# gau-nernst/vision-toolbox

Measured on AMD Instinct MI355X. Metric: images/sec (node) CSPDarknet-53 bf16 train step @224px, higher is better.
Workload: dtype bf16; 1 GPU; cspdarknet53 train step (fwd+CE+bwd+allreduce+SGD), batch 256/GPU, 3x224x224, 1000 classes, BASELINE configs[1]; global_batch=256, per_gpu_batch=256, parallelism=dp1, rccl_ranks=1, local_device=cuda:0, hip_graphs=False, main_stream_priority=-1, sync_bn=False, deterministic=False

## Files before the change

### vision-toolbox_amd/csrc/vt_pointwise.hip

```cpp
#include <stdlib.h>
#include <string.h>

#include <hip/hip_ext.h>

#include "vt_common.h"
#include "vt_bn_fin.h"

namespace {

typedef __attribute__((address_space(3))) s16x4 lds_s16x4;
typedef __attribute__((ext_vector_type(8))) short s16x8;

enum { PW_STATS = 0, PW_APPLY = 1, PW_REDUCE = 2, PW_BWD = 3 };

constexpr int pw_depth(int N, int K, int mode) {
#ifdef VT_PW_DEPTH
    return VT_PW_DEPTH;
#else
    return 1;
#endif
}

struct PwArgs {
    const bf16_t* x;
    int ldx;
    long M;
    int N0;
    const bf16_t* w[2];
    int ldw[2];
    bf16_t* y[2];
    const bf16_t* dy[2];
    int ldy[2];
    const bf16_t* res[2];
    int ldr[2];
    float* stats[2];
    const float* coef;
    const float* bcoef[2];
    bf16_t* dx;
    int lddx;
    const bf16_t* add;
    int ldadd;
    float* dw[2];
    int lddw[2];
    bf16_t* dz[2];
    int lddz[2];
    int relu;
    int nunits;
    int Nr, Kr;
    int fin;
    VtFinFwd ffin[2];
    VtFinBwd bfin[2];
    const float* pcoef;
    int pact;
    int pfin_on;
    VtFinFwd pfin;
    float* psums;
};

__device__ __forceinline__ uint4 ldg16(const bf16_t* p) { return *(const uint4*)p; }
__device__ __forceinline__ bf16x8 as_frag(const uint4& v) { return __builtin_bit_cast(bf16x8, v); }
__device__ __forceinline__ f32x4 mma(const bf16x8& a, const bf16x8& b, const f32x4& c) {
    return __builtin_amdgcn_mfma_f32_16x16x32_bf16(a, b, c, 0, 0, 0);
}
__device__ __forceinline__ float bfround(float v) { return (float)(bf16_t)v; }

template <int N, int K>
struct PwGeom {
    static constexpr int NT = N / 16, NU = N / 32, KS = K / 32, CT = K / 16, KV = K / 32;
    static constexpr int PITCH = 2 * K + 16;
    static constexpr int W_BYTES = N * PITCH;
    static constexpr int COEF_OFF = W_BYTES;
    static constexpr int RED_OFF = COEF_OFF + 5 * N * 4;
    static constexpr bool kFull = N * K <= 4096;
#ifndef VT_PW_REGW
#define VT_PW_REGW 2048
#endif
    static constexpr bool kRegW = N * K <= VT_PW_REGW;
    static constexpr int RED_BYTES = (kFull ? N * K * 4 : 0) > 4 * 2 * N * 4 ? N * K * 4 : 4 * 2 * N * 4;
    static constexpr int SMEM = RED_OFF + RED_BYTES;
};

template <int N, int K, int MODE, bool EX, int PROD = 0>
__global__ void __launch_bounds__(256) pw_kernel(const PwArgs a) {
    using G = PwGeom<N, K>;
    constexpr int NT = G::NT, NU = G::NU, KS = G::KS, CT = G::CT, KV = G::KV, PITCH = G::PITCH;
    constexpr bool kDW = (MODE == PW_BWD) && G::kFull;
    constexpr int kDepth = pw_depth(N, K, MODE);
    extern __shared__ __attribute__((aligned(16))) char smem[];
    char* sW = smem;
    float* sCoef = (float*)(smem + G::COEF_OFF);
    float* sRed = (float*)(smem + G::RED_OFF);

    const int tid = threadIdx.x, lane = tid & 63;
    const int wave = __builtin_amdgcn_readfirstlane(tid >> 6);
    const int pl = lane & 15, q = lane >> 4;
    const int N0 = a.N0;

    for (int idx = tid; idx < N * (K / 8); idx += 256) {
        const int n = idx / (K / 8), ch = idx - n * (K / 8);
        const int g = n >= N0;
        const bf16_t* src = a.w[g] + (long)(n - (g ? N0 : 0)) * a.ldw[g] + ch * 8;
        const bool real = n < a.Nr && ch * 8 < a.Kr;
        *(uint4*)(sW + n * PITCH + ch * 16) = real ? ldg16(src) : make_uint4(0, 0, 0, 0);
    }
    bool fin_done = false;
    if constexpr ((MODE == PW_APPLY || MODE == PW_BWD) && N <= 128) {
        if (a.fin) {
            fin_done = true;
            const int w = tid & 1, n = tid >> 1;
            const bool on = n < a.Nr;
            const int g = (on && n >= N0) ? 1 : 0, lc = on ? n - (g ? N0 : 0) : 0;
            if constexpr (MODE == PW_APPLY) {
                const VtFinFwd& f = a.ffin[g];
                const VtFinFwdPre pre = vt_fin_fwd_pre(f, lc);
                const double v = vt_replica_sum<false>(f.stats, (long)w * f.C + lc, 2L * f.C);
                const double o = __shfl_xor(v, 1, 64);
                if (on && w == 0) {
                    float sc, sf;
                    vt_fin_fwd_channel(f, lc, v, o, pre.g, pre.b, pre.rm, pre.rv, sc, sf, blockIdx.x == 0);
                    sCoef[n] = sc, sCoef[N + n] = sf;
                }
            } else {
                const VtFinBwd& f = a.bfin[g];
                const VtFinBwdPre pre = vt_fin_bwd_pre(f, lc);
                const float sh = on ? a.coef[N + n] : 0.f;
                const double v = vt_replica_sum<false>(f.sums, (long)w * f.C + lc, 2L * f.C);
                const double o = __shfl_xor(v, 1, 64);
                if (on && w == 0) {
                    float b, d;
                    vt_fin_bwd_channel(f, lc, v, o, pre.a, pre.mu, pre.istd, pre.dg, pre.db, b, d, blockIdx.x == 0);
                    sCoef[n] = pre.a, sCoef[N + n] = sh, sCoef[2 * N + n] = pre.a, sCoef[3 * N + n] = b, sCoef[4 * N + n] = d;
                }
            }
            for (int i = tid; i < 5 * N; i += 256) {
                const int which = i / N, n2 = i - which * N;
                if (n2 >= a.Nr || which >= (MODE == PW_APPLY ? 2 : 5)) sCoef[i] = 0.f;
// ... 50 lines not shown

    const unsigned za_base = (unsigned)((8 * (pl >> 2) + (pl & 3)) * PITCH + 16 * q);
    const unsigned ta_base = (unsigned)((8 * q + (pl >> 2)) * PITCH + 16 * (pl & 3));
    auto wz_frag = [&](int nt, int s) -> bf16x8 {
        const uint4 v = *(const uint4*)(sW + za_base + (nt >> 1) * 32 * PITCH + (nt & 1) * 4 * PITCH + s * 64);
        return as_frag(v);
    };
    auto wt_frag = [&](int ct, int u) -> bf16x8 {
        const char* p = sW + ta_base + u * 32 * PITCH + (ct >> 1) * 64 + (ct & 1) * 8;
        const s16x4 lo = __builtin_amdgcn_ds_read_tr16_b64_v4i16((lds_s16x4*)p);
        const s16x4 hi = __builtin_amdgcn_ds_read_tr16_b64_v4i16((lds_s16x4*)(p + 4 * PITCH));
        const s16x8 v = {lo[0], lo[1], lo[2], lo[3], hi[0], hi[1], hi[2], hi[3]};
        return __builtin_bit_cast(bf16x8, v);
    };
    bf16x8 wz[G::kRegW ? NT : 1][G::kRegW ? KS : 1];
    bf16x8 wt[(G::kRegW && MODE == PW_BWD) ? CT : 1][(G::kRegW && MODE == PW_BWD) ? NU : 1];
    if constexpr (G::kRegW) {
#pragma unroll
        for (int nt = 0; nt < NT; ++nt)
#pragma unroll
            for (int s = 0; s < KS; ++s) wz[nt][s] = wz_frag(nt, s);
        if constexpr (MODE == PW_BWD) {
#pragma unroll
            for (int ct = 0; ct < CT; ++ct)
#pragma unroll
                for (int u = 0; u < NU; ++u) wt[ct][u] = wt_frag(ct, u);
        }
    }
    bf16x8 sel[2];
    if constexpr (kDW) {
#pragma unroll
        for (int tt = 0; tt < 2; ++tt) {
            s16x8 v;
#pragma unroll
            for (int j = 0; j < 8; ++j) v[j] = (8 * q + j == 16 * tt + pl) ? (short)0x3F80 : (short)0;
            sel[tt] = __builtin_bit_cast(bf16x8, v);
        }
    }

    float s1[NU][8], s2[NU][8];
    if constexpr (MODE == PW_STATS || MODE == PW_REDUCE) {
#pragma unroll
        for (int u = 0; u < NU; ++u)
#pragma unroll
            for (int e = 0; e < 8; ++e) s1[u][e] = s2[u][e] = 0.f;
    }
    f32x4 dwacc[kDW ? NT : 1][kDW ? CT : 1];
    if constexpr (kDW) {
#pragma unroll
        for (int nt = 0; nt < NT; ++nt)
#pragma unroll
            for (int ct = 0; ct < CT; ++ct) dwacc[nt][ct] = f32x4{0.f, 0.f, 0.f, 0.f};
    }
    float p1[kPRed ? KV : 1][8], p2[kPRed ? KV : 1][8];
    if constexpr (kPRed) {
#pragma unroll
        for (int v = 0; v < KV; ++v)
#pragma unroll
            for (int e = 0; e < 8; ++e) p1[v][e] = p2[v][e] = 0.f;
    }

    struct Regs {
        uint4 x[KS];
        uint4 dy[(MODE >= PW_REDUCE) ? NU : 1];
        uint4 ex[(MODE == PW_APPLY) ? NU : (MODE == PW_BWD ? KV : 1)];
    };
    auto group_of = [&](int u) -> int { return 32 * u >= N0; };

    auto load_unit = [&](Regs& r, int unit) {
        const long p = (long)unit * 16 + pl;
        const long pc = p < a.M ? p : a.M - 1;
#pragma unroll
        for (int s = 0; s < KS; ++s) r.x[s] = ldg16(a.x + pc * a.ldx + (32 * s + 8 * q < a.Kr ? 32 * s + 8 * q : 0));
        if constexpr (MODE >= PW_REDUCE) {
#pragma unroll
            for (int u = 0; u < NU; ++u) {
                const int g = group_of(u);
                r.dy[u] = ldg16(a.dy[g] + pc * a.ldy[g] + (32 * u - (g ? N0 : 0)) + 8 * q);
            }
        }
        if constexpr (MODE == PW_APPLY) {
#pragma unroll
            for (int u = 0; u < NU; ++u) {
                const int g = group_of(u);
                if constexpr (EX)
                    r.ex[u] = ldg16(a.res[g] + pc * a.ldr[g] + (32 * u + 8 * q < a.Nr ? (32 * u - (g ? N0 : 0)) + 8 * q : 0));
            }
        }
        if constexpr (MODE == PW_BWD) {
            if constexpr (EX) {
#pragma unroll
                for (int v = 0; v < KV; ++v) r.ex[v] = ldg16(a.add + pc * a.ldadd + 32 * v + 8 * q);
            }
        }
    };

    auto compute_unit = [&](const Regs& r, int unit) {
        asm volatile("" ::: "memory");
        const long p = (long)unit * 16 + pl;
        const bool ok = p < a.M;
        uint4 xn[PROD ? KS : 1];
        if constexpr (PROD) {
#pragma unroll
            for (int s = 0; s < KS; ++s) {
                float v[8], psc[8], psf[8];
                const int ck = 32 * s + 8 * q;
                *(f32x4*)&psc[0] = *(const f32x4*)(sProd + ck);
                *(f32x4*)&psc[4] = *(const f32x4*)(sProd + ck + 4);
                *(f32x4*)&psf[0] = *(const f32x4*)(sProd + K + ck);
                *(f32x4*)&psf[4] = *(const f32x4*)(sProd + K + ck + 4);
                VecIO<bf16_t>::unpack(r.x[s], v);
#pragma unroll
                for (int e = 0; e < 8; ++e) {
                    v[e] = fmaf(v[e], psc[e], psf[e]);
                    v[e] = a.pact ? fmaxf(v[e], 0.f) : v[e];
                }
                xn[s] = VecIO<bf16_t>::pack(v);
            }
        }
        const uint4* xop = PROD ? xn : r.x;
        f32x4 zacc[NT];
#pragma unroll
        for (int nt = 0; nt < NT; ++nt) {
            zacc[nt] = f32x4{0.f, 0.f, 0.f, 0.f};
#pragma unroll
            for (int s = 0; s < KS; ++s) {
                const bf16x8 A = G::kRegW ? wz[G::kRegW ? nt : 0][G::kRegW ? s : 0] : wz_frag(nt, s);
                zacc[nt] = mma(A, as_frag(xop[s]), zacc[nt]);
            }
        }
        bf16x8 dzt[(MODE == PW_BWD) ? NU : 1];
#pragma unroll
        for (int u = 0; u < NU; ++u) {
            float z[8];
#pragma unroll
            for (int e = 0; e < 8; ++e) z[e] = bfround(zacc[2 * u + (e >> 2)][e & 3]);
            const int cb = 32 * u + 8 * q;
            if constexpr (MODE == PW_STATS) {
#pragma unroll
                for (int e = 0; e < 8; ++e) {
                    const float zz = ok ? z[e] : 0.f;
                    s1[u][e] += zz;
                    s2[u][e] = fmaf(zz, zz, s2[u][e]);
                }
            } else {
                float sc[8], sf[8];
                *(f32x4*)&sc[0] = *(const f32x4*)(sCoef + cb);
                *(f32x4*)&sc[4] = *(const f32x4*)(sCoef + cb + 4);
                *(f32x4*)&sf[0] = *(const f32x4*)(sCoef + N + cb);
                *(f32x4*)&sf[4] = *(const f32x4*)(sCoef + N + cb + 4);
                if constexpr (MODE == PW_APPLY) {
                    const int g = group_of(u);
                    float v[8], rr[8];
#pragma unroll
                    for (int e = 0; e < 8; ++e) rr[e] = 0.f;
                    if constexpr (EX) VecIO<bf16_t>::unpack(r.ex[u], rr);
#pragma unroll
                    for (int e = 0; e < 8; ++e) {
                        v[e] = fmaf(z[e], sc[e], sf[e]);
                        v[e] = a.relu ? fmaxf(v[e], 0.f) : v[e];
                        v[e] += rr[e];
                    }
                    if (ok && 32 * u + 8 * q < a.Nr)
                        *(uint4*)(a.y[g] + p * a.ldy[g] + (32 * u - (g ? N0 : 0)) + 8 * q) = VecIO<bf16_t>::pack(v);
                } else {
                    float gy[8];
                    VecIO<bf16_t>::unpack(r.dy[u], gy);
// ... 3 lines not shown
                        float mu[8];
                        *(f32x4*)&mu[0] = *(const f32x4*)(sCoef + 2 * N + cb);
                        *(f32x4*)&mu[4] = *(const f32x4*)(sCoef + 2 * N + cb + 4);
#pragma unroll
                        for (int e = 0; e < 8; ++e) {
                            s1[u][e] += gy[e];
                            s2[u][e] = fmaf(gy[e], z[e] - mu[e], s2[u][e]);
                        }
                    } else {
                        float ca[8], cbb[8], cd[8], dz[8];
                        *(f32x4*)&ca[0] = *(const f32x4*)(sCoef + 2 * N + cb);
                        *(f32x4*)&ca[4] = *(const f32x4*)(sCoef + 2 * N + cb + 4);
                        *(f32x4*)&cbb[0] = *(const f32x4*)(sCoef + 3 * N + cb);
                        *(f32x4*)&cbb[4] = *(const f32x4*)(sCoef + 3 * N + cb + 4);
                        *(f32x4*)&cd[0] = *(const f32x4*)(sCoef + 4 * N + cb);
                        *(f32x4*)&cd[4] = *(const f32x4*)(sCoef + 4 * N + cb + 4);
#pragma unroll
                        for (int e = 0; e < 8; ++e) {
                            dz[e] = fmaf(ca[e], gy[e], fmaf(-cbb[e], z[e], cd[e]));
                            dz[e] = ok ? dz[e] : 0.f;
                        }
                        const uint4 dzp = VecIO<bf16_t>::pack(dz);
                        dzt[u] = as_frag(dzp);
                        if constexpr (!kDW) {
                            const int g = group_of(u);
                            if (a.dz[g] && ok) *(uint4*)(a.dz[g] + p * a.lddz[g] + (32 * u - (g ? N0 : 0)) + 8 * q) = dzp;
                        }
                    }
                }
            }
        }
        if constexpr (MODE == PW_BWD) {
#pragma unroll
            for (int v = 0; v < KV; ++v) {
                f32x4 xa[2];
#pragma unroll
                for (int h = 0; h < 2; ++h) {
                    xa[h] = f32x4{0.f, 0.f, 0.f, 0.f};
#pragma unroll
                    for (int u = 0; u < NU; ++u) {
                        const bf16x8 A = G::kRegW ? wt[G::kRegW ? 2 * v + h : 0][G::kRegW ? u : 0] : wt_frag(2 * v + h, u);
                        xa[h] = mma(A, dzt[u], xa[h]);
                    }
                }
                float o[8], ad[8];
#pragma unroll
                for (int e = 0; e < 8; ++e) ad[e] = 0.f;
                if constexpr (EX) VecIO<bf16_t>::unpack(r.ex[v], ad);
#pragma unroll
                for (int e = 0; e < 8; ++e) o[e] = xa[e >> 2][e & 3] + ad[e];
                const uint4 dxp = VecIO<bf16_t>::pack(o);
                if (ok) *(uint4*)(a.dx + p * a.lddx + 32 * v + 8 * q) = dxp;
                if constexpr (kPRed) {
                    float gq[8], z0[8], psc[8], psf[8], pmu[8];
                    const int ck = 32 * v + 8 * q;
                    *(f32x4*)&psc[0] = *(const f32x4*)(sProd + ck);
                    *(f32x4*)&psc[4] = *(const f32x4*)(sProd + ck + 4);
                    *(f32x4*)&psf[0] = *(const f32x4*)(sProd + K + ck);
                    *(f32x4*)&psf[4] = *(const f32x4*)(sProd + K + ck + 4);
                    *(f32x4*)&pmu[0] = *(const f32x4*)(sProd + 2 * K + ck);
                    *(f32x4*)&pmu[4] = *(const f32x4*)(sProd + 2 * K + ck + 4);
                    VecIO<bf16_t>::unpack(dxp, gq);
                    VecIO<bf16_t>::unpack(r.x[v], z0);
#pragma unroll
                    for (int e = 0; e < 8; ++e) {
                        const float gg = (ok && (!a.pact || fmaf(z0[e], psc[e], psf[e]) > 0.f)) ? gq[e] : 0.f;
                        p1[v][e] += gg;
                        p2[v][e] = fmaf(gg, z0[e] - pmu[e], p2[v][e]);
                    }
                }
            }
        }
        if constexpr (kDW) {
            s16x4 dzT[NT], xT[CT];
            const f32x4 z4 = f32x4{0.f, 0.f, 0.f, 0.f};
#pragma unroll
            for (int nt = 0; nt < NT; ++nt) {
                const f32x4 t0 = mma(dzt[nt >> 1], sel[nt & 1], z4);
                const uint32_t lo = VecIO<bf16_t>::pack2(t0[0], t0[1]), hi = VecIO<bf16_t>::pack2(t0[2], t0[3]);
                dzT[nt] = __builtin_bit_cast(s16x4, make_uint2(lo, hi));
            }
#pragma unroll
            for (int ct = 0; ct < CT; ++ct) {
                const f32x4 t0 = mma(as_frag(xop[ct >> 1]), sel[ct & 1], z4);
                const uint32_t lo = VecIO<bf16_t>::pack2(t0[0], t0[1]), hi = VecIO<bf16_t>::pack2(t0[2], t0[3]);
                xT[ct] = __builtin_bit_cast(s16x4, make_uint2(lo, hi));
            }
#pragma unroll
            for (int nt = 0; nt < NT; ++nt)
#pragma unroll
                for (int ct = 0; ct < CT; ++ct)
                    dwacc[nt][ct] = __builtin_amdgcn_mfma_f32_16x16x16bf16_1k(dzT[nt], xT[ct], dwacc[nt][ct], 0, 0, 0);
        }
    };

    const int stride = (int)gridDim.x * 4;
    const int first = (int)blockIdx.x * 4 + wave;
    const int T = first < a.nunits ? (a.nunits - first + stride - 1) / stride : 0;
    if (T > 0) {
        auto unit_of = [&](int i) { return first + (i < T ? i : T - 1) * stride; };
        Regs ring[kDepth + 1];
#pragma unroll
        for (int j = 0; j < kDepth; ++j) load_unit(ring[j], unit_of(j));
        int i = 0;
        for (; i + kDepth + 1 <= T; i += kDepth + 1) {
#pragma unroll
            for (int j = 0; j <= kDepth; ++j) {
                load_unit(ring[(j + kDepth) % (kDepth + 1)], unit_of(i + j + kDepth));
                compute_unit(ring[j], first + (i + j) * stride);
            }
        }
#pragma unroll
        for (int j = 0; j < kDepth; ++j)
            if (i + j < T) compute_unit(ring[j], first + (i + j) * stride);
    }

    if constexpr (MODE == PW_STATS || MODE == PW_REDUCE) {
#pragma unroll
        for (int u = 0; u < NU; ++u)
#pragma unroll
            for (int e = 0; e < 8; ++e) {
#pragma unroll
                for (int off = 1; off < 16; off <<= 1) {
                    s1[u][e] += __shfl_xor(s1[u][e], off, 64);
                    s2[u][e] += __shfl_xor(s2[u][e], off, 64);
                }
            }
        if (pl == 0) {
#pragma unroll
            for (int u = 0; u < NU; ++u)
#pragma unroll
                for (int e = 0; e < 8; ++e) {
                    sRed[(wave * 2 + 0) * N + 32 * u + 8 * q + e] = s1[u][e];
                    sRed[(wave * 2 + 1) * N + 32 * u + 8 * q + e] = s2[u][e];
                }
        }
        __syncthreads();
        const int rep = (int)(blockIdx.x % kStatReplicas);
        for (int i = tid; i < 2 * N; i += 256) {
            const int which = i / N, n = i - which * N;
            float acc = sRed[(0 * 2 + which) * N + n];
            acc += sRed[(1 * 2 + which) * N + n];
            acc += sRed[(2 * 2 + which) * N + n];
            acc += sRed[(3 * 2 + which) * N + n];
            if (MODE == PW_REDUCE && which) acc *= sCoef[3 * N + n];
            const int g = n >= N0, Cg = g ? N - N0 : N0, c = n - (g ? N0 : 0);
            vt_stat_add(a.stats[g], ((long)rep * 2 + which) * Cg + c, acc);
        }
    }
    if constexpr (kDW) {
#pragma unroll
        for (int nt = 0; nt < NT; ++nt)
#pragma unroll
            for (int ct = 0; ct < CT; ++ct)
#pragma unroll
                for (int r = 0; r < 4; ++r) atomicAdd(&sRed[(16 * nt + 4 * q + r) * K + 16 * ct + pl], dwacc[nt][ct][r]);
        __syncthreads();
        constexpr int NCH = N * K / 256;
        const int rot = (int)((blockIdx.x * 7u) % (unsigned)NCH);
        for (int j = 0; j < NCH; ++j) {
            int ch = j + rot;
            ch -= ch >= NCH ? NCH : 0;
            const int i = ch * 256 + tid;
            const int n = i / K, c = i - n * K;
            const int g = n >= N0;
            float* dst = a.dw[g];
            if (dst) atomicAdd(dst + (long)(n - (g ? N0 : 0)) * a.lddw[g] + c, sRed[i]);
        }
    }
    if constexpr (kPRed) {
#pragma unroll
        for (int v = 0; v < KV; ++v)
#pragma unroll
            for (int e = 0; e < 8; ++e) {
#pragma unroll
                for (int off = 1; off < 16; off <<= 1) {
                    p1[v][e] += __shfl_xor(p1[v][e], off, 64);
                    p2[v][e] += __shfl_xor(p2[v][e], off, 64);
                }
            }
        __syncthreads();
        if (pl == 0) {
#pragma unroll
            for (int v = 0; v < KV; ++v)
#pragma unroll
                for (int e = 0; e < 8; ++e) {
                    sRed[(wave * 2 + 0) * K + 32 * v + 8 * q + e] = p1[v][e];
                    sRed[(wave * 2 + 1) * K + 32 * v + 8 * q + e] = p2[v][e];
                }
        }
        __syncthreads();
        const int rep = (int)(blockIdx.x % kStatReplicas);
        for (int i = tid; i < 2 * K; i += 256) {
            const int which = i / K, c = i - which * K;
            float acc = sRed[(0 * 2 + which) * K + c];
            acc += sRed[(1 * 2 + which) * K + c];
            acc += sRed[(2 * 2 + which) * K + c];
            acc += sRed[(3 * 2 + which) * K + c];
            if (which) acc *= sProd[3 * K + c];
            vt_stat_add(a.psums, ((long)rep * 2 + which) * K + c, acc);
        }
    }
}

template <int N, int K, int MODE, bool EX, int PROD = 0>
int launch_pw(const PwArgs& a, hipStream_t st, const char* who) {
    using G = PwGeom<N, K>;
    auto kern = pw_kernel<N, K, MODE, EX, PROD>;
    constexpr int smem = G::SMEM + (PROD ? 4 * K * 4 : 0);
    static_assert(smem <= 160 * 1024, "weights exceed the LDS of a CU");
    if (smem > 64 * 1024) {
        const int rc = vt_raise_dynamic_lds((const void*)kern, smem, who);
        if (rc != VT_OK) return rc;
    }
    const int knob = (0);
    const int target = knob > 0 ? knob : (a.nunits >= 160000 ? 768 : 512);
    const int per_wave = (8);
    long blocks = ((long)a.nunits + 4 * per_wave - 1) / (4 * per_wave);
    if (blocks > target) blocks = target;
    if (blocks < 1) blocks = 1;
    vt_note_kernel(PROD == 2 ? "pw_kernel<%d,%d,%s,prod+sums>" : PROD ? "pw_kernel<%d,%d,%s,prod>" : "pw_kernel<%d,%d,%s>", N, K, MODE == PW_STATS ? "stats" : MODE == PW_APPLY ? "apply" : MODE == PW_REDUCE ? "reduce" : "bwd");
    VT_LAUNCH_STOP(kern, dim3((unsigned)blocks), dim3(256), smem, st, a);
    VT_CHECK_LAUNCH(who);
    return VT_OK;
}

template <int MODE>
int dispatch_pw(int N, int K, const PwArgs& a, hipStream_t st, const char* who) {
    const bool ex = MODE == PW_APPLY ? a.res[0] != nullptr : (MODE == PW_BWD ? a.add != nullptr : false);
    if (a.pcoef) {
#define VT_PW_PROD_CASE(n, k)                                                      \
    if (N == n && K == k) {                                                        \
        if constexpr (MODE == PW_APPLY || MODE == PW_BWD) {                        \
            if (ex) return launch_pw<n, k, MODE, true, 1>(a, st, who);             \
        }                                                                          \
        if constexpr (MODE == PW_BWD) {                                            \
            if (a.psums) return launch_pw<n, k, MODE, false, 2>(a, st, who);       \
        }                                                                          \
        return launch_pw<n, k, MODE, false, 1>(a, st, who);                        \
    }
        VT_PW_PROD_CASE(32, 32)
        VT_PW_PROD_CASE(64, 64)
        VT_PW_PROD_CASE(32, 64)
#undef VT_PW_PROD_CASE
        vt_set_error("%s: no pointwise kernel with a producer operand for %d -> %d channels", who, K, N);
        return VT_ERR_UNSUPPORTED;
    }
#define VT_PW_CASE(n, k)                                                           \
    if (N == n && K == k) {                                                        \
        if constexpr (MODE == PW_APPLY || MODE == PW_BWD) {                        \
            if (ex) return launch_pw<n, k, MODE, true>(a, st, who);                \
        }                                                                          \
        return launch_pw<n, k, MODE, false>(a, st, who);                           \
    }
    VT_PW_CASE(32, 32)
    VT_PW_CASE(64, 64)
    VT_PW_CASE(32, 64)
    VT_PW_CASE(128, 128)
    VT_PW_CASE(64, 128)
    VT_PW_CASE(160, 160)
    VT_PW_CASE(160, 320)
#undef VT_PW_CASE
// ... 5 lines not shown
    return VT_ERR_UNSUPPORTED;
}

bool shape_ok(int N, int K) {
    return (N == 32 && K == 32) || (N == 64 && K == 64) || (N == 32 && K == 64) || (N == 128 && K == 128) ||
           (N == 64 && K == 128) || (N == 160 && K == 160) || (N == 160 && K == 320);
}

bool ragged_apply_ok(int N, int K, int ngroups) { return ngroups == 1 && N == 80 && (K == 80 || K == 160); }

int fill_common(PwArgs& a, const vt_pw_desc* d, const char* who, bool apply = false) {
    VT_REQUIRE(d, VT_ERR_INVALID, "%s: null descriptor", who);
    VT_REQUIRE(d->dtype == VT_BF16, VT_ERR_UNSUPPORTED, "%s: bf16 only", who);
    VT_REQUIRE(d->M > 0 && d->M < 0x7fffffffL * 16, VT_ERR_INVALID, "%s: bad M", who);
    VT_REQUIRE(d->ngroups == 1 || d->ngroups == 2, VT_ERR_INVALID, "%s: ngroups %d", who, d->ngroups);
    const int N = d->C[0] + (d->ngroups == 2 ? d->C[1] : 0);
    const bool ragged = apply && ragged_apply_ok(N, d->K, d->ngroups);
    VT_REQUIRE(ragged || shape_ok(N, d->K), VT_ERR_UNSUPPORTED, "%s: no pointwise kernel for %d -> %d channels", who, d->K, N);
    VT_REQUIRE(ragged || (d->C[0] > 0 && d->C[0] % 32 == 0 && (d->ngroups == 1 || (d->C[1] > 0 && d->C[1] % 32 == 0))),
               VT_ERR_UNSUPPORTED, "%s: group widths must be multiples of 32", who);
    VT_REQUIRE(d->x && vt_aligned16(d->x) && d->ldx % 8 == 0 && d->ldx >= d->K, VT_ERR_INVALID, "%s: bad x", who);
    VT_REQUIRE(d->M * (int64_t)d->ldx < 0x7fffffff00LL, VT_ERR_UNSUPPORTED, "%s: tensor too large", who);
    memset(&a, 0, sizeof(a));
    a.x = (const bf16_t*)d->x;
    a.ldx = d->ldx;
    a.M = d->M;
    a.N0 = d->C[0];
    a.relu = d->relu;
    a.nunits = (int)((d->M + 15) / 16);
    a.Nr = N, a.Kr = d->K;
    for (int g = 0; g < d->ngroups; ++g) {
        VT_REQUIRE(d->w[g] && vt_aligned16(d->w[g]) && d->ldw[g] % 8 == 0 && d->ldw[g] >= d->K, VT_ERR_INVALID,
                   "%s: bad weights of group %d", who, g);
        a.w[g] = (const bf16_t*)d->w[g];
        a.ldw[g] = d->ldw[g];
    }
    if (d->pcoef) {
        VT_REQUIRE(!ragged && (int64_t)N * d->K <= 4096, VT_ERR_UNSUPPORTED,
                   "%s: a producer operand needs a shape with vt_pw_supported() == 2 (%d -> %d channels)", who, d->K, N);
        VT_REQUIRE(d->pact == 0 || d->pact == 1, VT_ERR_UNSUPPORTED, "%s: producer activation code %d (0 / 1 only)", who, d->pact);
        VT_REQUIRE(vt_aligned16(d->pcoef), VT_ERR_INVALID, "%s: bad producer coefficients", who);
        a.pcoef = d->pcoef;
        a.pact = d->pact;
    }
    return VT_OK;
}

int check_rows(const char* who, const char* what, int g, const void* p, int ld, int C, bool optional) {
    if (!p && optional) return VT_OK;
    VT_REQUIRE(p && vt_aligned16(p) && ld % 8 == 0 && ld >= C, VT_ERR_INVALID, "%s: bad %s of group %d", who, what, g);
    return VT_OK;
}

}

extern "C" {

int vt_pw_supported(int32_t dtype, int32_t K, int32_t C0, int32_t C1) {
    if (dtype != VT_BF16 || C0 <= 0 || C1 < 0 || C0 % 32 != 0 || C1 % 32 != 0) return 0;
    const int N = C0 + C1;
    if (!shape_ok(N, K)) return 0;
    return N * K <= 4096 ? 2 : 1;
}

int vt_pw_apply_supported(int32_t dtype, int32_t K, int32_t C0) {
    return dtype == VT_BF16 && (shape_ok(C0, K) || ragged_apply_ok(C0, K, 1));
}

static int pw_fwd_stats_impl(const vt_pw_desc* d, const vt_bn_fin_fwd* pfin, float* const* stats, void* stream) {
    PwArgs a;
    int rc = fill_common(a, d, "vt_pw_fwd_stats");
    if (rc != VT_OK) return rc;
    for (int g = 0; g < d->ngroups; ++g) {
        VT_REQUIRE(stats && stats[g], VT_ERR_INVALID, "vt_pw_fwd_stats: null statistics buffer");
        a.stats[g] = stats[g];
    }
    if (pfin) {
        float* c = (float*)d->pcoef;
        const int K = d->K;
        a.pfin_on = 1;
        a.pfin = VtFinFwd{pfin->stats, pfin->gamma, pfin->beta, pfin->running_mean, pfin->running_var, pfin->num_batches_tracked,
                          c, c + K, c + 2 * K, c + 3 * K, 1.0 / pfin->count,
                          pfin->count > 1.0 ? pfin->count / (pfin->count - 1.0) : 1.0, pfin->eps, pfin->momentum, K};
    }
    return dispatch_pw<PW_STATS>(a.N0 + (d->ngroups == 2 ? d->C[1] : 0), d->K, a, (hipStream_t)stream, "vt_pw_fwd_stats");
}

int vt_pw_fwd_stats(const vt_pw_desc* d, float* const* stats, void* stream) { return pw_fwd_stats_impl(d, nullptr, stats, stream); }

int vt_pw_fwd_stats_finalize(const vt_pw_desc* d, const vt_bn_fin_fwd* pfin, float* const* stats, void* stream) {
    VT_REQUIRE(d && pfin, VT_ERR_INVALID, "vt_pw_fwd_stats_finalize: null argument");
    VT_REQUIRE(d->pcoef, VT_ERR_INVALID, "vt_pw_fwd_stats_finalize: the descriptor has no producer operand");
    VT_REQUIRE(pfin->stats && pfin->count > 0, VT_ERR_INVALID, "vt_pw_fwd_stats_finalize: bad statistics of the producer");
    VT_REQUIRE((pfin->running_mean == nullptr) == (pfin->running_var == nullptr), VT_ERR_INVALID,
               "vt_pw_fwd_stats_finalize: running_mean/var must both be given or both NULL");
    if (!VT_KNOB("VT_BN_FIN_APPLY", 1)) {
        float* c = (float*)d->pcoef;
        const int K = d->K;
        const int rc = vt_bn_finalize(pfin->stats, K, pfin->count, pfin->gamma, pfin->beta, pfin->eps, pfin->momentum,
                                      pfin->running_mean, pfin->running_var, pfin->num_batches_tracked, c, c + K, c + 2 * K,
                                      c + 3 * K, stream);
        if (rc != VT_OK) return rc;
        return pw_fwd_stats_impl(d, nullptr, stats, stream);
    }
    return pw_fwd_stats_impl(d, pfin, stats, stream);
}
// ... 168 lines not shown
```

### vision-toolbox_amd/csrc/vt_igemm.hip

```cpp
#include <stdlib.h>

#include "vt_common.h"
#include "vt_igemm_args.h"

namespace {

constexpr int kTapBytes = VT_MAX_TAPS * 16;
constexpr int stat_bytes(int WM, int BN) { return WM * 2 * BN * 4 > 2048 ? WM * 2 * BN * 4 : 2048; }

__device__ __attribute__((aligned(16))) unsigned int vt_zero16[4];

__device__ __forceinline__ int swz(int row) { return (0x1320 >> (((row >> 2) & 3) * 4)) & 3; }

__device__ __forceinline__ void glds16(const void* gsrc, unsigned lds_base) {
    unsigned keep;
    asm volatile(
        "s_mov_b32 %0, m0\n\t"
        "s_mov_b32 m0, %2\n\t"
        "s_nop 0\n\t"
        "global_load_lds_dwordx4 %1, off\n\t"
        "s_mov_b32 m0, %0"
        : "=&s"(keep)
        : "v"(gsrc), "s"(lds_base)
        : "memory");
// ... 412 lines not shown
    VT_REQUIRE(d->Cin % epc == 0 && d->Cout % epc == 0 && d->ldx % epc == 0 && d->ldy % epc == 0 &&
                   d->ldw % epc == 0,
               VT_ERR_UNSUPPORTED,
               "vt_conv_igemm: Cin=%d Cout=%d ldx=%d ldy=%d ldw=%d must be multiples of %d", d->Cin,
               d->Cout, d->ldx, d->ldy, d->ldw, epc);
    const bool d2s = (d->flags & VT_CONV_D2S) != 0;
    if (d2s) {
        VT_REQUIRE(d->Cout % (4 * epc) == 0 && d->oHs == 2 && d->oWs == 2 && d->oh0 == 0 && d->ow0 == 0 &&
                       d->oH == 2 * d->Ho && d->oW == 2 * d->Wo &&
                       !(d->flags & (VT_CONV_STATS | VT_CONV_AFFINE | VT_CONV_RELU)),
                   VT_ERR_UNSUPPORTED, "vt_conv_igemm: D2S needs Cout = 4*C', a 2x2-strided output and a raw epilogue");
    }
    VT_REQUIRE(d->ldx >= d->Cin && d->ldy >= (d2s ? d->Cout / 4 : d->Cout) && d->ldw >= d->ntaps * d->Cin, VT_ERR_INVALID,
               "vt_conv_igemm: stride smaller than extent");
    VT_REQUIRE(vt_aligned16(x) && vt_aligned16(w) && vt_aligned16(y), VT_ERR_INVALID,
               "vt_conv_igemm: x/w/y must be 16-byte aligned");
    VT_REQUIRE(d->oHs >= 1 && d->oWs >= 1 && d->oh0 >= 0 && d->ow0 >= 0 &&
                   (d->Ho - 1) * d->oHs + d->oh0 < d->oH && (d->Wo - 1) * d->oWs + d->ow0 < d->oW,
               VT_ERR_INVALID, "vt_conv_igemm: output placement outside the %dx%d tensor", d->oH, d->oW);
    const long in_elems = (long)d->B * d->Hi * d->Wi * d->ldx;
    const long out_elems = (long)d->B * d->oH * d->oW * d->ldy;
    VT_REQUIRE(in_elems < 0x7fffffffL && out_elems < 0x7fffffffL && (long)d->B * d->Ho * d->Wo < 0x7fffffffL,
               VT_ERR_UNSUPPORTED, "vt_conv_igemm: tensor exceeds 2^31 elements");
    if (d->flags & VT_CONV_RESIDUAL) {
        VT_REQUIRE(residual && vt_aligned16(residual) && d->ldr % epc == 0 && d->ldr >= (d2s ? d->Cout / 4 : d->Cout),
                   VT_ERR_INVALID, "vt_conv_igemm: bad residual");
    }
    if (d->flags & VT_CONV_AFFINE) VT_REQUIRE(shift, VT_ERR_INVALID, "vt_conv_igemm: AFFINE needs shift");
    if (d->flags & VT_CONV_STATS) {
        VT_REQUIRE(stats, VT_ERR_INVALID, "vt_conv_igemm: STATS needs a stats buffer");
        VT_REQUIRE(!(d->flags & (VT_CONV_AFFINE | VT_CONV_RELU | VT_CONV_RESIDUAL)), VT_ERR_UNSUPPORTED,
                   "vt_conv_igemm: STATS is only defined on the raw conv output");
    }

    IgemmArgs a;
    fill_args(a, d, x, w, y, scale, shift, residual, stats);

    hipStream_t st = (hipStream_t)stream;
    if (!d2s) {
        const int rc = vt_stem_dispatch(a, d->dtype, stream);
        if (rc >= 0) return rc;
        const int rc6 = vt_stem6_dispatch(a, d->dtype, stream);
        if (rc6 >= 0) return rc6;
    }
    VT_REQUIRE(!(d->flags & VT_CONV_NOSTORE), VT_ERR_UNSUPPORTED, "vt_conv_igemm: NOSTORE outside the RGB stem kernel");
    if (!d2s) {
        const int rc = vt_span6_dispatch(a, d->dtype, stream);
        if (rc >= 0) return rc;
    }
    {
        const int rc = vt_pspan_dispatch(a, d->dtype, stream);
        if (rc >= 0) return rc;
    }
    {
        const int rc = vt_span_dispatch(a, d->dtype, stream);
        if (rc >= 0) return rc;
    }
    if (d->dtype == VT_BF16) {
        const int w8 = VT_KNOB("VT_IGEMM_W8", 3);
        if (VT_KNOB("VT_IGEMM_BN80", 1) && d->Cout % 80 == 0 && d->Cout <= 160) {
            if ((w8 & 1) && d->Cout == 160) return launch<bf16_t, 256, 160, 4, 2, 2>(a, st);
            return launch<bf16_t, 256, 80, 4, 1, 2>(a, st);
        }
        if (d->Cout > 64 && (w8 & 2) && ((long)(a.M + 255) / 256) * ((d->Cout + 127) / 128) >= ((w8 & 4) ? 0 : 256))
            return launch<bf16_t, 256, 128, 4, 2, 2>(a, st);
        if (d->Cout > 64) return launch<bf16_t, 128, 128, 2, 2, 2>(a, st);
        if (d->Cout > 32) return launch<bf16_t, 128, 64, 2, 2, 2>(a, st);
        return launch<bf16_t, 256, 32, 4, 1, 2>(a, st);
    }
    if (d->Cout > 32) return launch<float, 128, 64, 2, 2, 2>(a, st);
    return launch<float, 128, 32, 4, 1, 2>(a, st);
}

extern "C" int vt_conv_dgrad_bnred(const vt_conv_desc* d, const void* dz, const void* w, void* dy, const void* z, int32_t ldz,
                                   const float* scale, const float* shift, const float* mean, const float* invstd,
                                   int32_t relu, float* sums, void* stream) {
    VT_REQUIRE(d && dz && w && dy && z && scale && shift && mean && invstd && sums, VT_ERR_INVALID,
               "vt_conv_dgrad_bnred: null argument");
    VT_REQUIRE(relu == 0 || relu == 1, VT_ERR_UNSUPPORTED, "vt_conv_dgrad_bnred: activation code %d (none / ReLU only)", relu);
    VT_REQUIRE(d->flags == 0, VT_ERR_INVALID, "vt_conv_dgrad_bnred: the launch has a plain epilogue (flags 0x%x)", d->flags);
    const long M = (long)d->B * d->oH * d->oW;
    const bool whole = d->oHs == 1 && d->oWs == 1 && d->oh0 == 0 && d->ow0 == 0 && d->oH == d->Ho && d->oW == d->Wo;
    VT_REQUIRE(whole, VT_ERR_INVALID, "vt_conv_dgrad_bnred: the launch must produce every pixel of d(y)");
    const int epc = vt_epc(d->dtype);
    VT_REQUIRE(ldz % epc == 0 && ldz >= d->Cout && vt_aligned16(z), VT_ERR_INVALID, "vt_conv_dgrad_bnred: bad z");
    if (d->dtype == VT_BF16 && VT_KNOB("VT_DGRAD_BNRED", 1) && d->ntaps >= 1 && d->ntaps <= VT_MAX_TAPS && d->Cin % epc == 0 &&
        d->Cout % epc == 0 && d->ldx % epc == 0 && d->ldy % epc == 0 && d->ldw % epc == 0 && d->ldx >= d->Cin &&
        d->ldy >= d->Cout && d->ldw >= d->ntaps * d->Cin && vt_aligned16(dz) && vt_aligned16(w) && vt_aligned16(dy) &&
        (long)d->B * d->Hi * d->Wi * d->ldx < 0x7fffffffL && M * d->ldy < 0x7fffffffL && M * ldz < 0x7fffffffL) {
        IgemmArgs a;
        fill_args(a, d, dz, w, dy, scale, shift, z, sums);
        a.ldr = ldz;
        a.aux0 = mean, a.aux1 = invstd;
        a.flags = VT_CONV_BNRED | (relu ? VT_CONV_RELU : 0);
        const int rc = vt_span6_dispatch(a, d->dtype, stream);
        if (rc >= 0) return rc;
    }
    const int rc = vt_conv_igemm(d, dz, w, dy, nullptr, nullptr, nullptr, nullptr, stream);
    if (rc != VT_OK) return rc;
    return vt_bn_act_bwd_reduce(dy, d->ldy, z, ldz, scale, shift, mean, invstd, M, d->Cout, relu, d->dtype, sums, stream);
}
```

### vision-toolbox_amd/csrc/vt_igemm_args.h

```cpp
#pragma once
#include "vt_common.h"

#define VT_CONV_BNRED 0x1000

#ifndef VT_MFMA_SETPRIO
#define VT_MFMA_SETPRIO 0
#endif

struct IgemmArgs {
    const void* x;
    const void* w;
    void* y;
    const float* scale;
    const float* shift;
    const void* res;
    float* stats;
    int B, Hi, Wi, Cin, ldx, Ho, Wo, sh, sw, h0, w0, Cout, ldy, oH, oW, oHs, oWs, oh0, ow0;
    int ldw, ldr, flags, ntaps;
    int M, Ktot, tiles_m, tiles_n, chunk, dense_out;
    int fast_dma;
    int8_t dh[VT_MAX_TAPS];
    int8_t dw[VT_MAX_TAPS];
    const float* aux0;
    const float* aux1;
};

__device__ __forceinline__ long vt_out_col(const IgemmArgs& p, int n, int ld) {
    if (!(p.flags & VT_CONV_D2S)) return n;
    const int cq = p.Cout >> 2;
    const int blk = n / cq;
    return ((long)(blk >> 1) * p.oW + (blk & 1)) * ld + (n - blk * cq);
}

int vt_span_dispatch(IgemmArgs& a, int dtype, void* stream);

int vt_span6_dispatch(IgemmArgs& a, int dtype, void* stream);

int vt_pspan_dispatch(IgemmArgs& a, int dtype, void* stream);

int vt_stem_dispatch(IgemmArgs& a, int dtype, void* stream);

int vt_stem6_dispatch(IgemmArgs& a, int dtype, void* stream);
```

Before: 13330 images/sec.

## Compress producer-BN gradient partial sums via DPP scatter-reduce and reuse relu mask

In the fused pointwise backward kernel with producer-BN sums (PROD==2), the per-lane 2x8xKV partial-sum accumulators are replaced by one register per KV chunk. Each step's 16 values are reduced across the 16-lane row with a DPP scatter-sum. The ReLU/validity mask is recorded during the forward recompute, so the scale/shift reloads and the FMA recheck go away. The end-of-block shuffle reduction and its two barriers are dropped in favour of a dedicated LDS slot, and the kernel gets a waves-per-eu hint. The aim is lower register pressure and better occupancy, at the cost of per-unit DPP work and extra LDS.

```diff
diff --git a/vision-toolbox_amd/csrc/vt_pointwise.hip b/vision-toolbox_amd/csrc/vt_pointwise.hip
--- a/vision-toolbox_amd/csrc/vt_pointwise.hip
+++ b/vision-toolbox_amd/csrc/vt_pointwise.hip
@@ -64,6 +64,26 @@
 }
 __device__ __forceinline__ float bfround(float v) { return (float)(bf16_t)v; }
 
+template <int CTRL>
+__device__ __forceinline__ float pw_dpp(float v) {
+    return __builtin_bit_cast(float, __builtin_amdgcn_update_dpp(0, __builtin_bit_cast(int, v), CTRL, 0xf, 0xf, false));
+}
+template <int H, int CTRL>
+__device__ __forceinline__ void pw_scatter_step(float* t, bool hi) {
+#pragma unroll
+    for (int i = 0; i < H; ++i) {
+        const float keep = hi ? t[H + i] : t[i], send = hi ? t[i] : t[H + i];
+        t[i] = keep + pw_dpp<CTRL>(send);
+    }
+}
+__device__ __forceinline__ float pw_row_scatter_sum(float (&t)[16], int pl) {
+    pw_scatter_step<8, 0x128>(t, pl & 8);
+    pw_scatter_step<4, 0x141>(t, pl & 4);
+    pw_scatter_step<2, 0x4E>(t, pl & 2);
+    pw_scatter_step<1, 0xB1>(t, pl & 1);
+    return t[0];
+}
+
 template <int N, int K>
 struct PwGeom {
     static constexpr int NT = N / 16, NU = N / 32, KS = K / 32, CT = K / 16, KV = K / 32;
@@ -81,7 +101,7 @@
 };
 
 template <int N, int K, int MODE, bool EX, int PROD = 0>
-__global__ void __launch_bounds__(256) pw_kernel(const PwArgs a) {
+__global__ void __launch_bounds__(256) __attribute__((amdgpu_waves_per_eu(PROD == 2 ? 2 : 1))) pw_kernel(const PwArgs a) {
     using G = PwGeom<N, K>;
     constexpr int NT = G::NT, NU = G::NU, KS = G::KS, CT = G::CT, KV = G::KV, PITCH = G::PITCH;
     constexpr bool kDW = (MODE == PW_BWD) && G::kFull;
@@ -238,12 +258,10 @@
 #pragma unroll
             for (int ct = 0; ct < CT; ++ct) dwacc[nt][ct] = f32x4{0.f, 0.f, 0.f, 0.f};
     }
-    float p1[kPRed ? KV : 1][8], p2[kPRed ? KV : 1][8];
+    float ps[kPRed ? KV : 1];
     if constexpr (kPRed) {
 #pragma unroll
-        for (int v = 0; v < KV; ++v)
-#pragma unroll
-            for (int e = 0; e < 8; ++e) p1[v][e] = p2[v][e] = 0.f;
+        for (int v = 0; v < KV; ++v) ps[v] = 0.f;
     }
 
     struct Regs {
@@ -286,9 +304,11 @@
         const long p = (long)unit * 16 + pl;
         const bool ok = p < a.M;
         uint4 xn[PROD ? KS : 1];
+        unsigned pmask[PROD == 2 ? KS : 1];
         if constexpr (PROD) {
 #pragma unroll
             for (int s = 0; s < KS; ++s) {
+                if constexpr (PROD == 2) pmask[s] = 0u;
                 float v[8], psc[8], psf[8];
                 const int ck = 32 * s + 8 * q;
                 *(f32x4*)&psc[0] = *(const f32x4*)(sProd + ck);
@@ -299,6 +319,7 @@
 #pragma unroll
                 for (int e = 0; e < 8; ++e) {
                     v[e] = fmaf(v[e], psc[e], psf[e]);
+                    if constexpr (PROD == 2) pmask[s] |= (ok && (!a.pact || v[e] > 0.f)) ? 1u << e : 0u;
                     v[e] = a.pact ? fmaxf(v[e], 0.f) : v[e];
                 }
                 xn[s] = VecIO<bf16_t>::pack(v);
@@ -408,22 +429,20 @@
                 const uint4 dxp = VecIO<bf16_t>::pack(o);
                 if (ok) *(uint4*)(a.dx + p * a.lddx + 32 * v + 8 * q) = dxp;
                 if constexpr (kPRed) {
-                    float gq[8], z0[8], psc[8], psf[8], pmu[8];
+                    float gq[8], z0[8], pmu[8];
                     const int ck = 32 * v + 8 * q;
-                    *(f32x4*)&psc[0] = *(const f32x4*)(sProd + ck);
-                    *(f32x4*)&psc[4] = *(const f32x4*)(sProd + ck + 4);
-                    *(f32x4*)&psf[0] = *(const f32x4*)(sProd + K + ck);
-                    *(f32x4*)&psf[4] = *(const f32x4*)(sProd + K + ck + 4);
                     *(f32x4*)&pmu[0] = *(const f32x4*)(sProd + 2 * K + ck);
                     *(f32x4*)&pmu[4] = *(const f32x4*)(sProd + 2 * K + ck + 4);
                     VecIO<bf16_t>::unpack(dxp, gq);
                     VecIO<bf16_t>::unpack(r.x[v], z0);
+                    float t[16];
 #pragma unroll
                     for (int e = 0; e < 8; ++e) {
-                        const float gg = (ok && (!a.pact || fmaf(z0[e], psc[e], psf[e]) > 0.f)) ? gq[e] : 0.f;
-                        p1[v][e] += gg;
-                        p2[v][e] = fmaf(gg, z0[e] - pmu[e], p2[v][e]);
+                        const float gg = (pmask[v] >> e & 1u) ? gq[e] : 0.f;
+                        t[e] = gg;
+                        t[8 + e] = gg * (z0[e] - pmu[e]);
                     }
+                    ps[v] += pw_row_scatter_sum(t, pl);
                 }
             }
         }
@@ -503,6 +522,11 @@
             const int g = n >= N0, Cg = g ? N - N0 : N0, c = n - (g ? N0 : 0);
             vt_stat_add(a.stats[g], ((long)rep * 2 + which) * Cg + c, acc);
         }
+    }
+    float* sPSum = sProd + 4 * K;
+    if constexpr (kPRed) {
+#pragma unroll
+        for (int v = 0; v < KV; ++v) sPSum[(wave * 2 + (pl >> 3)) * K + 32 * v + 8 * q + (pl & 7)] = ps[v];
     }
     if constexpr (kDW) {
 #pragma unroll
@@ -525,34 +549,13 @@
         }
     }
     if constexpr (kPRed) {
-#pragma unroll
-        for (int v = 0; v < KV; ++v)
-#pragma unroll
-            for (int e = 0; e < 8; ++e) {
-#pragma unroll
-                for (int off = 1; off < 16; off <<= 1) {
-                    p1[v][e] += __shfl_xor(p1[v][e], off, 64);
-                    p2[v][e] += __shfl_xor(p2[v][e], off, 64);
-                }
-            }
-        __syncthreads();
-        if (pl == 0) {
-#pragma unroll
-            for (int v = 0; v < KV; ++v)
-#pragma unroll
-                for (int e = 0; e < 8; ++e) {
-                    sRed[(wave * 2 + 0) * K + 32 * v + 8 * q + e] = p1[v][e];
-                    sRed[(wave * 2 + 1) * K + 32 * v + 8 * q + e] = p2[v][e];
-                }
-        }
-        __syncthreads();
         const int rep = (int)(blockIdx.x % kStatReplicas);
         for (int i = tid; i < 2 * K; i += 256) {
             const int which = i / K, c = i - which * K;
-            float acc = sRed[(0 * 2 + which) * K + c];
-            acc += sRed[(1 * 2 + which) * K + c];
-            acc += sRed[(2 * 2 + which) * K + c];
-            acc += sRed[(3 * 2 + which) * K + c];
+            float acc = sPSum[(0 * 2 + which) * K + c];
+            acc += sPSum[(1 * 2 + which) * K + c];
+            acc += sPSum[(2 * 2 + which) * K + c];
+            acc += sPSum[(3 * 2 + which) * K + c];
             if (which) acc *= sProd[3 * K + c];
             vt_stat_add(a.psums, ((long)rep * 2 + which) * K + c, acc);
         }
@@ -563,7 +566,7 @@
 int launch_pw(const PwArgs& a, hipStream_t st, const char* who) {
     using G = PwGeom<N, K>;
     auto kern = pw_kernel<N, K, MODE, EX, PROD>;
-    constexpr int smem = G::SMEM + (PROD ? 4 * K * 4 : 0);
+    constexpr int smem = G::SMEM + (PROD ? 4 * K * 4 : 0) + (PROD == 2 ? 4 * 2 * K * 4 : 0);
     static_assert(smem <= 160 * 1024, "weights exceed the LDS of a CU");
     if (smem > 64 * 1024) {
         const int rc = vt_raise_dynamic_lds((const void*)kern, smem, who);
```

After: 13390 images/sec, median of 6. No clear change (+0.5%).

## Add weight-stationary pointwise 1x1 conv kernel for measured bf16 shapes

Applied to the files above, without the earlier changes.

Adds a dedicated 1x1 stride-1 convolution kernel that keeps the whole weight slice in LDS and streams 16-row units of the activation per wave, double-buffered in registers. It applies only to a table of measured K/N/M shapes and skips stats epilogues unless forced. It can fuse a residual add. The aim is to beat the generic implicit-GEMM and span kernels on the large pointwise convs of CSPDarknet by reusing weights and avoiding the im2col machinery. The cost is another kernel path to maintain and possible regressions on shapes where the general kernel was better tuned.

```diff
diff --git a/vision-toolbox_amd/csrc/vt_igemm.hip b/vision-toolbox_amd/csrc/vt_igemm.hip
--- a/vision-toolbox_amd/csrc/vt_igemm.hip
+++ b/vision-toolbox_amd/csrc/vt_igemm.hip
@@ -488,6 +488,10 @@
         const int rc = vt_pspan_dispatch(a, d->dtype, stream);
         if (rc >= 0) return rc;
     }
+    if (!d2s) {
+        const int rc = vt_pwconv_dispatch(a, d->dtype, stream);
+        if (rc >= 0) return rc;
+    }
     {
         const int rc = vt_span_dispatch(a, d->dtype, stream);
         if (rc >= 0) return rc;
diff --git a/vision-toolbox_amd/csrc/vt_igemm_args.h b/vision-toolbox_amd/csrc/vt_igemm_args.h
--- a/vision-toolbox_amd/csrc/vt_igemm_args.h
+++ b/vision-toolbox_amd/csrc/vt_igemm_args.h
@@ -38,6 +38,8 @@
 
 int vt_pspan_dispatch(IgemmArgs& a, int dtype, void* stream);
 
+int vt_pwconv_dispatch(IgemmArgs& a, int dtype, void* stream);
+
 int vt_stem_dispatch(IgemmArgs& a, int dtype, void* stream);
 
 int vt_stem6_dispatch(IgemmArgs& a, int dtype, void* stream);
diff --git a/vision-toolbox_amd/csrc/vt_pointwise.hip b/vision-toolbox_amd/csrc/vt_pointwise.hip
--- a/vision-toolbox_amd/csrc/vt_pointwise.hip
+++ b/vision-toolbox_amd/csrc/vt_pointwise.hip
@@ -5,6 +5,7 @@
 
 #include "vt_common.h"
 #include "vt_bn_fin.h"
+#include "vt_igemm_args.h"
 
 namespace {
 
@@ -675,6 +676,249 @@
     return VT_OK;
 }
 
+enum { EPI_PLAIN = 0, EPI_STATS = 1, EPI_RES = 2 };
+
+struct PwConvArgs {
+    const bf16_t* x;
+    const bf16_t* w;
+    bf16_t* y;
+    const bf16_t* res;
+    float* stats;
+    long M;
+    int ldx, ldw, ldy, ldr;
+    int N;
+    int nunits;
+};
+
+template <int BN, int K>
+struct PwConvGeom {
+    static constexpr int NT = BN / 16, NU = BN / 32, KS = K / 32;
+    static constexpr int PITCH = 2 * K + 16;
+    static constexpr int RED_OFF = BN * PITCH;
+    static constexpr int SMEM = RED_OFF + 4 * 2 * BN * 4;
+};
+
+template <int BN, int K, int EPI>
+__global__ void __launch_bounds__(256) pw_conv_kernel(const PwConvArgs a) {
+    using G = PwConvGeom<BN, K>;
+    constexpr int NT = G::NT, NU = G::NU, KS = G::KS, PITCH = G::PITCH;
+    extern __shared__ __attribute__((aligned(16))) char smem[];
+    char* sW = smem;
+    float* sRed = (float*)(smem + G::RED_OFF);
+
+    const int tid = threadIdx.x, lane = tid & 63;
+    const int wave = __builtin_amdgcn_readfirstlane(tid >> 6);
+    const int pl = lane & 15, q = lane >> 4;
+    const int n0 = (int)blockIdx.y * BN;
+
+    for (int idx = tid; idx < BN * (K / 8); idx += 256) {
+        const int n = idx / (K / 8), ch = idx - n * (K / 8);
+        *(uint4*)(sW + n * PITCH + ch * 16) = ldg16(a.w + (long)(n0 + n) * a.ldw + ch * 8);
+    }
+    __syncthreads();
+
+    const unsigned za_base = (unsigned)((8 * (pl >> 2) + (pl & 3)) * PITCH + 16 * q);
+    auto wz_frag = [&](int nt, int s) -> bf16x8 {
+        const uint4 v = *(const uint4*)(sW + za_base + (nt >> 1) * 32 * PITCH + (nt & 1) * 4 * PITCH + s * 64);
+        return as_frag(v);
+    };
+
+    float s1[EPI == EPI_STATS ? NU : 1][8], s2[EPI == EPI_STATS ? NU : 1][8];
+    if constexpr (EPI == EPI_STATS) {
+#pragma unroll
+        for (int u = 0; u < NU; ++u)
+#pragma unroll
+            for (int e = 0; e < 8; ++e) s1[u][e] = s2[u][e] = 0.f;
+    }
+
+    struct Regs {
+        uint4 x[KS];
+        uint4 ex[EPI == EPI_RES ? NU : 1];
+    };
+    auto load_unit = [&](Regs& r, int unit) {
+        const long p = (long)unit * 16 + pl;
+        const long pc = p < a.M ? p : a.M - 1;
+#pragma unroll
+        for (int s = 0; s < KS; ++s) r.x[s] = ldg16(a.x + pc * a.ldx + 32 * s + 8 * q);
+        if constexpr (EPI == EPI_RES) {
+#pragma unroll
+            for (int u = 0; u < NU; ++u) r.ex[u] = ldg16(a.res + pc * a.ldr + n0 + 32 * u + 8 * q);
+        }
+    };
+    auto compute_unit = [&](const Regs& r, int unit) {
+        asm volatile("" ::: "memory");
+        const long p = (long)unit * 16 + pl;
+        const bool ok = p < a.M;
+        f32x4 zacc[NT];
+#pragma unroll
+        for (int nt = 0; nt < NT; ++nt) {
+            zacc[nt] = f32x4{0.f, 0.f, 0.f, 0.f};
+#pragma unroll
+            for (int s = 0; s < KS; ++s) zacc[nt] = mma(wz_frag(nt, s), as_frag(r.x[s]), zacc[nt]);
+        }
+#pragma unroll
+        for (int u = 0; u < NU; ++u) {
+            float z[8];
+#pragma unroll
+            for (int e = 0; e < 8; ++e) z[e] = bfround(zacc[2 * u + (e >> 2)][e & 3]);
+            if constexpr (EPI == EPI_RES) {
+                float rr[8];
+                VecIO<bf16_t>::unpack(r.ex[u], rr);
+#pragma unroll
+                for (int e = 0; e < 8; ++e) z[e] += rr[e];
+            }
+            if constexpr (EPI == EPI_STATS) {
+#pragma unroll
+                for (int e = 0; e < 8; ++e) {
+                    const float zz = ok ? z[e] : 0.f;
+                    s1[u][e] += zz;
+                    s2[u][e] = fmaf(zz, zz, s2[u][e]);
+                }
+            }
+            if (ok) *(uint4*)(a.y + p * a.ldy + n0 + 32 * u + 8 * q) = VecIO<bf16_t>::pack(z);
+        }
+    };
+
+    const int stride = (int)gridDim.x * 4;
+    const int first = (int)blockIdx.x * 4 + wave;
+    const int T = first < a.nunits ? (a.nunits - first + stride - 1) / stride : 0;
+    if (T > 0) {
+        auto unit_of = [&](int i) { return first + (i < T ? i : T - 1) * stride; };
+        Regs ring[2];
+        load_unit(ring[0], unit_of(0));
+        int i = 0;
+        for (; i + 2 <= T; i += 2) {
+            load_unit(ring[1], unit_of(i + 1));
+            compute_unit(ring[0], first + i * stride);
+            load_unit(ring[0], unit_of(i + 2));
+            compute_unit(ring[1], first + (i + 1) * stride);
+        }
+        if (i < T) compute_unit(ring[0], first + i * stride);
+    }
+
+    if constexpr (EPI == EPI_STATS) {
+#pragma unroll
+        for (int u = 0; u < NU; ++u)
+#pragma unroll
+            for (int e = 0; e < 8; ++e) {
+#pragma unroll
+                for (int off = 1; off < 16; off <<= 1) {
+                    s1[u][e] += __shfl_xor(s1[u][e], off, 64);
+                    s2[u][e] += __shfl_xor(s2[u][e], off, 64);
+                }
+            }
+        if (pl == 0) {
+#pragma unroll
+            for (int u = 0; u < NU; ++u)
+#pragma unroll
+                for (int e = 0; e < 8; ++e) {
+                    sRed[(wave * 2 + 0) * BN + 32 * u + 8 * q + e] = s1[u][e];
+                    sRed[(wave * 2 + 1) * BN + 32 * u + 8 * q + e] = s2[u][e];
+                }
+        }
+        __syncthreads();
+        const int rep = (int)(blockIdx.x % kStatReplicas);
+        for (int i = tid; i < 2 * BN; i += 256) {
+            const int which = i / BN, n = i - which * BN;
+            float acc = sRed[(0 * 2 + which) * BN + n];
+            acc += sRed[(1 * 2 + which) * BN + n];
+            acc += sRed[(2 * 2 + which) * BN + n];
+            acc += sRed[(3 * 2 + which) * BN + n];
+            vt_stat_add(a.stats, ((long)rep * 2 + which) * a.N + n0 + n, acc);
+        }
+    }
+}
+
+int pwconv_row_blocks(int nunits, int tiles_n) {
+    const int forced = VT_KNOB("VT_PWCONV_GX", 0);
+    if (forced > 0) return forced < 65536 ? forced : 65535;
+    const int knob = VT_KNOB("VT_PWCONV_WPC", 0);
+    const int wpc = knob > 0 ? knob : 1;
+    int cus = vt_device_cus();
+    if (cus <= 0) cus = 256;
+    long gx = ((long)cus * wpc + tiles_n - 1) / tiles_n;
+    const long most = ((long)nunits + 3) / 4;
+    if (gx > most) gx = most;
+    if (gx >= 8) gx = gx / 8 * 8;
+    return gx < 1 ? 1 : (int)gx;
+}
+
+template <int BN, int K>
+int launch_pwconv(const PwConvArgs& a, int epi, hipStream_t st) {
+    using G = PwConvGeom<BN, K>;
+    static_assert(2 * G::SMEM <= 160 * 1024, "two workgroups per CU");
+    void (*kern)(const PwConvArgs) = epi == EPI_STATS ? pw_conv_kernel<BN, K, EPI_STATS>
+                                     : epi == EPI_RES ? pw_conv_kernel<BN, K, EPI_RES>
+                                                      : pw_conv_kernel<BN, K, EPI_PLAIN>;
+    if (G::SMEM > 64 * 1024) {
+        const int rc = vt_raise_dynamic_lds((const void*)kern, G::SMEM, "vt_conv_igemm(pwconv)");
+        if (rc != VT_OK) return rc;
+    }
+    const int tiles_n = a.N / BN;
+    const int gx = pwconv_row_blocks(a.nunits, tiles_n);
+    vt_note_kernel("pw_conv_kernel<bf16,%d,%d,%s>", BN, K, epi == EPI_STATS ? "stats" : epi == EPI_RES ? "res" : "plain");
+    hipLaunchKernelGGL(kern, dim3((unsigned)gx, (unsigned)tiles_n), dim3(256), G::SMEM, st, a);
+    VT_CHECK_LAUNCH("vt_conv_igemm(pwconv)");
+    return VT_OK;
+}
+
+struct PwConvClass {
+    int K, N;
+    long Mmin, Mmax;
+};
+constexpr PwConvClass kPwConvTable[] = {
+    {128, 128, 200704, 200704},
+    {256, 128, 200704, 200704},
+    {128, 256, 200704, 200704},
+    {256, 256, 200704, 200704},
+    {256, 256, 50176, 50176},
+    {256, 512, 50176, 50176},
+};
+
+bool pwconv_measured(int K, int N, long M) {
+    for (const PwConvClass& c : kPwConvTable)
+        if (c.K == K && c.N == N && M >= c.Mmin && M <= c.Mmax) return true;
+    return false;
+}
+
+}
+
+int vt_pwconv_dispatch(IgemmArgs& a, int dtype, void* stream) {
+    const int enabled = VT_KNOB("VT_PWCONV", 1);
+    if (!enabled || dtype != VT_BF16) return -1;
+    if (a.ntaps != 1 || a.sh != 1 || a.sw != 1 || a.h0 + a.dh[0] != 0 || a.w0 + a.dw[0] != 0) return -1;
+    if (a.Ho != a.Hi || a.Wo != a.Wi || !a.dense_out) return -1;
+    if (a.flags & ~(VT_CONV_STATS | VT_CONV_RESIDUAL)) return -1;
+    if ((a.flags & VT_CONV_STATS) && (a.flags & VT_CONV_RESIDUAL)) return -1;
+    if (a.ldx % 8 || a.ldy % 8 || a.ldw % 8 || ((a.flags & VT_CONV_RESIDUAL) && a.ldr % 8)) return -1;
+    const int K = a.Cin, N = a.Cout;
+    if ((K != 128 && K != 256 && K != 512) || N % 64 != 0 || N > 64 * 65535) return -1;
+    if (enabled < 2 && !pwconv_measured(K, N, a.M)) return -1;
+    if (enabled < 2 && (a.flags & VT_CONV_STATS)) return -1;
+    if ((a.flags & VT_CONV_RESIDUAL) && a.res) {
+        const char* y0 = (const char*)a.y;
+        const char* y1 = y0 + ((long)(a.M - 1) * a.ldy + N) * 2;
+        const char* r0 = (const char*)a.res;
+        const char* r1 = r0 + ((long)(a.M - 1) * a.ldr + N) * 2;
+        if (r0 < y1 && y0 < r1 && !(r0 == y0 && a.ldr == a.ldy)) {
+            const long cb = (long)N * 2, pitch = (long)a.ldy * 2;
+            long off = (r0 - y0) % pitch;
+            if (off < 0) off += pitch;
+            if (!(a.ldr == a.ldy && off >= cb && off + cb <= pitch)) return -1;
+        }
+    }
+    PwConvArgs c;
+    memset(&c, 0, sizeof(c));
+    c.x = (const bf16_t*)a.x, c.w = (const bf16_t*)a.w, c.y = (bf16_t*)a.y;
+    c.res = (a.flags & VT_CONV_RESIDUAL) ? (const bf16_t*)a.res : nullptr;
+    c.stats = a.stats;
+    c.M = a.M, c.ldx = a.ldx, c.ldw = a.ldw, c.ldy = a.ldy, c.ldr = a.ldr, c.N = N;
+    c.nunits = (int)(((long)a.M + 15) / 16);
+    const int epi = (a.flags & VT_CONV_STATS) ? EPI_STATS : (c.res ? EPI_RES : EPI_PLAIN);
+    hipStream_t st = (hipStream_t)stream;
+    if (K == 128) return N % 128 == 0 ? launch_pwconv<128, 128>(c, epi, st) : launch_pwconv<64, 128>(c, epi, st);
+    if (K == 256) return N % 128 == 0 ? launch_pwconv<128, 256>(c, epi, st) : launch_pwconv<64, 256>(c, epi, st);
+    return launch_pwconv<64, 512>(c, epi, st);
 }
 
 extern "C" {
```

Result: no change. 13350 images/sec before, 13380 images/sec after, median of 6 (+0.3%).
